# Brummi/MonoRec

Hardware: AMD Instinct MI355X
Metric: frames/sec (keyframes/s), KITTI 256x512 2-src/32-bin cost-volume inference (higher is better)
Workload: dtype f32

## Files before the change

### include/monorec_hip.h

```cpp
#ifndef MONOREC_HIP_H
#define MONOREC_HIP_H

#include <stddef.h>
#include <stdint.h>

#ifdef __cplusplus
extern "C" {
#endif

#define MR_ABI_VERSION 21

#define MR_COMPUTE_F32  0
#define MR_COMPUTE_BF16 1
#define MR_COMPUTE_BF16X3 2

#define MR_ERR_BAD_ARGUMENT (-1)
#define MR_ERR_UNSUPPORTED  (-2)
#define MR_ERR_LDS_BUDGET   (-3)

#define MR_MAX_SOURCES 3
#define MR_MAX_FRAMES  8
#define MR_MAX_HEADS   4
#define MR_MAX_VOTE_MASKS 8

enum {
    MR_ACT_NONE = 0,
    MR_ACT_RELU = 1,
    MR_ACT_LEAKY_RELU = 2,
    MR_ACT_SIGMOID = 3,
    MR_ACT_ABS_TANH_AFFINE = 4
};

enum {
    MR_IN_DIRECT = 0,
    MR_IN_UPSAMPLE2 = 1,
    MR_IN_MAXPOOL2 = 2
};

enum {
    MR_TF_NONE = 0,
    MR_TF_RESNET_NORM = 1
};

// ... 127 lines not shown
int mr_conv2d_b8(const mr_b8_conv_desc* desc, void* stream);
int mr_pool2x2_framemax_b8(const void* src, void* pooled, void* fmax, int32_t frames, int64_t planes, int32_t h, int32_t w, void* stream);
int mr_max_over_frames_b8(const void* src, void* dst, int32_t frames, int64_t groups16, void* stream);
int mr_cost_volume_b8_f32(const float* keyframe, const float* const* frames, int32_t num_frames, const float* kinv, const float* proj,
                          const float* depths, int32_t batch, int32_t num_depths, int32_t height, int32_t width, float alpha,
                          const float* channel_weights, int32_t use_ssim, const float* pixel_depths, float* cost_volume,
                          float* const* sfcv, void* const* sfcv_b8, void* stream);
int mr_cost_volume_b8_lean_f32(const float* keyframe, const float* const* frames, int32_t num_frames, const float* kinv, const float* proj,
                               const float* depths, int32_t batch, int32_t num_depths, int32_t height, int32_t width, float alpha,
                               const float* channel_weights, int32_t use_ssim, const float* pixel_depths, float* cost_volume,
                               float* const* sfcv_scratch, void* const* sfcv_b8, void* stream);
int mr_mask_classifier_b8_f32(const float* features, const float* weight, const float* bias, int32_t batch, int32_t channels, int64_t plane,
                              float* cv_mask, float* cost_volume, int32_t num_depths, void* cost_volume_b8, void* stream);
int mr_f32_nchw_to_b8(const float* src, void* dst, int32_t n, int32_t c, int64_t hw, void* stream);
int mr_b8_to_f32_nchw(const void* src, float* dst, int32_t n, int32_t c, int64_t hw, void* stream);

size_t mr_wino1d_packed_weight_floats(int32_t out_channels, const int32_t* src_channels, int32_t num_src, int32_t cout_blocks_per_wave);
int mr_wino1d_pack_weights_f32(const float* weight, int32_t out_channels, const int32_t* src_channels, int32_t num_src,
                               int32_t cout_blocks_per_wave, float* dst);
int64_t mr_conv1d3_winograd_lds_bytes(const mr_wino_desc* desc);
int mr_conv1d3_winograd_f32(const mr_wino_desc* desc, int32_t axis, void* stream);

size_t mr_cooktoom1d_packed_weight_floats(int32_t out_channels, const int32_t* src_channels, int32_t num_src, int32_t cout_blocks_per_wave,
                                          int32_t m, int32_t r);
int mr_cooktoom1d_pack_weights_f32(const float* weight, int32_t out_channels, const int32_t* src_channels, int32_t num_src,
                                   int32_t cout_blocks_per_wave, int32_t m, int32_t r, float* dst);
int64_t mr_conv1d_cooktoom_lds_bytes(const mr_wino_desc* desc, int32_t axis, int32_t m, int32_t r);
int mr_conv1d_cooktoom_f32(const mr_wino_desc* desc, int32_t axis, int32_t m, int32_t r, void* stream);

int mr_upconv_pack_weights_f32(const float* weight, int32_t out_channels, const int32_t* src_channels, int32_t num_src,
                               int32_t cout_blocks_per_wave, float* dst);
int mr_upconv2x2_winograd_f32(const mr_wino_desc* desc, void* stream);

size_t mr_wino_t_packed_weight_floats(int32_t out_channels, const int32_t* src_channels, int32_t num_src, int32_t cout_blocks_per_wave);
int mr_wino_t_pack_weights_f32(const float* weight, int32_t out_channels, const int32_t* src_channels, int32_t num_src,
                               int32_t cout_blocks_per_wave, float* dst);
size_t mr_wino_t_packed_weight_floats_tail(int32_t out_channels, const int32_t* src_channels, int32_t num_src);
int mr_wino_t_pack_weights_tail_f32(const float* weight, int32_t out_channels, const int32_t* src_channels, int32_t num_src, float* dst);
int64_t mr_convt4x4s2_winograd_lds_bytes(const mr_wino_desc* desc);
int mr_convt4x4s2_winograd_f32(const mr_wino_desc* desc, void* stream);

int mr_cost_volume_f32(const float* keyframe, const float* const* frames, int32_t num_frames,
                       const float* kinv, const float* proj, const float* depths,
                       int32_t batch, int32_t num_depths, int32_t height, int32_t width,
                       float alpha, const float* channel_weights ,
                       float* cost_volume, float* const* sfcv, void* stream);

int mr_cost_volume_mode_f32(const float* keyframe, const float* const* frames, int32_t num_frames,
                            const float* kinv, const float* proj, const float* depths,
                            int32_t batch, int32_t num_depths, int32_t height, int32_t width,
                            float alpha, const float* channel_weights, int32_t use_ssim,
                            const float* pixel_depths, int32_t sfcv_mult_mask,
                            float* cost_volume, float* const* sfcv, void* stream);

int mr_cost_volume_relaxed_f32(const float* keyframe, const float* const* frames, int32_t num_frames,
                               const float* kinv, const float* proj, const float* depths,
                               int32_t batch, int32_t num_depths, int32_t height, int32_t width,
                               float alpha, const float* channel_weights, int32_t use_ssim, const float* pixel_depths,
                               float* cost_volume, float* const* sfcv, void* stream);

int mr_cost_volume_tiled_f32(const float* keyframe, const float* const* frames, int32_t num_frames,
                             const float* kinv, const float* proj, const float* depths,
                             int32_t batch, int32_t num_depths, int32_t height, int32_t width,
                             float alpha, const float* channel_weights, int32_t use_ssim,
                             const float* pixel_depths, int32_t sfcv_mult_mask,
                             float* cost_volume, float* const* sfcv, void* stream);
// ... 132 lines not shown
```

### monorec_amd/_lib.py

```python
import ctypes
import os

MR_MAX_SOURCES = 3
MR_MAX_FRAMES = 8

ACT_NONE, ACT_RELU, ACT_LEAKY_RELU, ACT_SIGMOID, ACT_ABS_TANH_AFFINE = range(5)
IN_DIRECT, IN_UPSAMPLE2, IN_MAXPOOL2 = range(3)
TF_NONE, TF_RESNET_NORM = range(2)

_c_float_p = ctypes.POINTER(ctypes.c_float)


class ConvDesc(ctypes.Structure):
    _fields_ = [
        ("src", ctypes.c_void_p * MR_MAX_SOURCES),
        ("src_channels", ctypes.c_int32 * MR_MAX_SOURCES),
        ("num_src", ctypes.c_int32),
        ("batch", ctypes.c_int32),
        ("src_h", ctypes.c_int32), ("src_w", ctypes.c_int32),
        ("in_mode", ctypes.c_int32),
        ("in_transform", ctypes.c_int32),
        ("kh", ctypes.c_int32), ("kw", ctypes.c_int32),
        ("stride_h", ctypes.c_int32), ("stride_w", ctypes.c_int32),
        ("pad_top", ctypes.c_int32), ("pad_left", ctypes.c_int32),
# ... 24 lines not shown
        ("k_split_waves", ctypes.c_int32),
    ]


class WinoDesc(ctypes.Structure):
    _fields_ = [("src", ctypes.c_void_p * MR_MAX_SOURCES), ("src_channels", ctypes.c_int32 * MR_MAX_SOURCES), ("num_src", ctypes.c_int32),
                ("batch", ctypes.c_int32), ("height", ctypes.c_int32), ("width", ctypes.c_int32),
                ("dst", ctypes.c_void_p), ("out_channels", ctypes.c_int32),
                ("packed_weights", ctypes.c_void_p), ("bias", ctypes.c_void_p), ("residual", ctypes.c_void_p),
                ("activation", ctypes.c_int32), ("act_p0", ctypes.c_float), ("cout_blocks_per_wave", ctypes.c_int32),
                ("variant", ctypes.c_int32),
                ("src_row_pitch", ctypes.c_int32), ("src_plane_floats", ctypes.c_int32), ("dst_split_columns", ctypes.c_int32)]


LAYOUT_F32_NCHW, LAYOUT_BF16_B8 = 0, 1


class B8ConvDesc(ctypes.Structure):
    _fields_ = [("src", ctypes.c_void_p * MR_MAX_SOURCES), ("src_channels", ctypes.c_int32 * MR_MAX_SOURCES), ("src_layout", ctypes.c_int32 * MR_MAX_SOURCES),
                ("num_src", ctypes.c_int32), ("batch", ctypes.c_int32), ("src_h", ctypes.c_int32), ("src_w", ctypes.c_int32),
                ("kh", ctypes.c_int32), ("kw", ctypes.c_int32), ("stride_h", ctypes.c_int32), ("stride_w", ctypes.c_int32),
                ("out_h", ctypes.c_int32), ("out_w", ctypes.c_int32),
                ("dst", ctypes.c_void_p), ("dst_layout", ctypes.c_int32), ("out_channels", ctypes.c_int32),
                ("dst_plane_h", ctypes.c_int32), ("dst_plane_w", ctypes.c_int32), ("out_step_h", ctypes.c_int32), ("out_step_w", ctypes.c_int32),
                ("bias", ctypes.c_void_p), ("activation", ctypes.c_int32), ("act_p0", ctypes.c_float),
                ("cout_blocks_per_wg", ctypes.c_int32), ("pixel_blocks_per_wave", ctypes.c_int32), ("waves_per_wg", ctypes.c_int32),
                ("num_phases", ctypes.c_int32),
                ("phase_weights", ctypes.c_void_p * 4), ("phase_kh", ctypes.c_int32 * 4), ("phase_kw", ctypes.c_int32 * 4),
                ("phase_pad_top", ctypes.c_int32 * 4), ("phase_pad_left", ctypes.c_int32 * 4),
                ("phase_out_off_h", ctypes.c_int32 * 4), ("phase_out_off_w", ctypes.c_int32 * 4)]


MR_MAX_COPY_SEGMENTS = 24
MR_ABI_VERSION = 21


class CopySegment(ctypes.Structure):
    _fields_ = [("src", ctypes.c_void_p), ("dst", ctypes.c_void_p), ("bytes", ctypes.c_int64)]


class LaunchItem(ctypes.Structure):
    _fields_ = [("kind", ctypes.c_int32), ("arg", ctypes.c_int32), ("desc", ctypes.c_void_p)]


LAUNCH_CONV2D, LAUNCH_WINO3X3, LAUNCH_WINO_T, LAUNCH_WINO_1D, LAUNCH_UPCONV, LAUNCH_COOKTOOM_1D, LAUNCH_WINO44, LAUNCH_CONV_B8, LAUNCH_WINO44S, LAUNCH_WINO44W = 0, 1, 2, 3, 4, 5, 6, 7, 8, 9


class HeadDesc(ctypes.Structure):
    _fields_ = [("src", ctypes.c_void_p), ("weight", ctypes.c_void_p), ("bias", ctypes.c_void_p), ("dst", ctypes.c_void_p),
                ("batch", ctypes.c_int32), ("channels", ctypes.c_int32), ("height", ctypes.c_int32), ("width", ctypes.c_int32)]


MR_MAX_HEADS = 4

ABI = {
    "mr_conv_packed_weight_floats": (ctypes.c_size_t, [ctypes.c_int32, ctypes.POINTER(ctypes.c_int32), ctypes.c_int32,
                                                       ctypes.c_int32, ctypes.c_int32, ctypes.c_int32, ctypes.c_int32]),
    "mr_conv_pack_weights_f32": (ctypes.c_int, [ctypes.c_void_p, ctypes.c_int32, ctypes.POINTER(ctypes.c_int32),
                                                ctypes.c_int32, ctypes.c_int32, ctypes.c_int32, ctypes.c_int32,
                                                ctypes.c_int32, ctypes.c_void_p]),
    "mr_conv_packed_weight_floats_bf16": (ctypes.c_size_t, [ctypes.c_int32, ctypes.POINTER(ctypes.c_int32), ctypes.c_int32,
                                                            ctypes.c_int32, ctypes.c_int32, ctypes.c_int32, ctypes.c_int32]),
    "mr_conv_packed_weight_floats_bf16x3": (ctypes.c_size_t, [ctypes.c_int32, ctypes.POINTER(ctypes.c_int32), ctypes.c_int32,
                                                              ctypes.c_int32, ctypes.c_int32, ctypes.c_int32, ctypes.c_int32]),
    "mr_conv_pack_weights_bf16x3": (ctypes.c_int, [ctypes.c_void_p, ctypes.c_int32, ctypes.POINTER(ctypes.c_int32),
                                                    ctypes.c_int32, ctypes.c_int32, ctypes.c_int32, ctypes.c_int32, ctypes.c_int32,
                                                    ctypes.c_void_p]),
# ... 16 lines not shown
                                          ctypes.c_void_p, ctypes.c_void_p, ctypes.c_void_p,
                                          ctypes.c_int32, ctypes.c_int32, ctypes.c_int32, ctypes.c_int32,
                                          ctypes.c_float, _c_float_p,
                                          ctypes.c_void_p, ctypes.POINTER(ctypes.c_void_p), ctypes.c_void_p]),
    "mr_cost_volume_mode_f32": (ctypes.c_int, [ctypes.c_void_p, ctypes.POINTER(ctypes.c_void_p), ctypes.c_int32,
                                               ctypes.c_void_p, ctypes.c_void_p, ctypes.c_void_p,
                                               ctypes.c_int32, ctypes.c_int32, ctypes.c_int32, ctypes.c_int32,
                                               ctypes.c_float, _c_float_p, ctypes.c_int32, ctypes.c_void_p, ctypes.c_int32,
                                               ctypes.c_void_p, ctypes.POINTER(ctypes.c_void_p), ctypes.c_void_p]),
    "mr_cost_volume_relaxed_f32": (ctypes.c_int, [ctypes.c_void_p, ctypes.POINTER(ctypes.c_void_p), ctypes.c_int32,
                                                  ctypes.c_void_p, ctypes.c_void_p, ctypes.c_void_p,
                                                  ctypes.c_int32, ctypes.c_int32, ctypes.c_int32, ctypes.c_int32,
                                                  ctypes.c_float, _c_float_p, ctypes.c_int32, ctypes.c_void_p,
                                                  ctypes.c_void_p, ctypes.POINTER(ctypes.c_void_p), ctypes.c_void_p]),
    "mr_cost_volume_tiled_f32": (ctypes.c_int, [ctypes.c_void_p, ctypes.POINTER(ctypes.c_void_p), ctypes.c_int32,
                                                ctypes.c_void_p, ctypes.c_void_p, ctypes.c_void_p,
                                                ctypes.c_int32, ctypes.c_int32, ctypes.c_int32, ctypes.c_int32,
                                                ctypes.c_float, _c_float_p, ctypes.c_int32, ctypes.c_void_p, ctypes.c_int32,
                                                ctypes.c_void_p, ctypes.POINTER(ctypes.c_void_p), ctypes.c_void_p]),
    "mr_cost_volume_patch_f32": (ctypes.c_int, [ctypes.c_void_p, ctypes.POINTER(ctypes.c_void_p), ctypes.c_int32,
                                                ctypes.c_void_p, ctypes.c_void_p, ctypes.c_void_p,
                                                ctypes.c_int32, ctypes.c_int32, ctypes.c_int32, ctypes.c_int32,
                                                ctypes.c_float, _c_float_p, ctypes.c_int32, ctypes.c_void_p, ctypes.c_int32, ctypes.c_int32,
                                                ctypes.c_void_p, ctypes.POINTER(ctypes.c_void_p), ctypes.c_void_p]),
    "mr_maxpool3x3s2_f32": (ctypes.c_int, [ctypes.c_void_p, ctypes.c_void_p, ctypes.c_int32, ctypes.c_int32,
                                           ctypes.c_int32, ctypes.c_void_p]),
    "mr_maxpool2x2_f32": (ctypes.c_int, [ctypes.c_void_p, ctypes.c_void_p, ctypes.c_int64, ctypes.c_int32,
                                         ctypes.c_int32, ctypes.c_void_p]),
    "mr_resnet_normalize_f32": (ctypes.c_int, [ctypes.c_void_p, ctypes.c_void_p, ctypes.c_int64, ctypes.c_void_p]),
    "mr_exact_const_division": (ctypes.c_int, [ctypes.c_float]),
    "mr_run_launches": (ctypes.c_int, [ctypes.POINTER(LaunchItem), ctypes.c_int32, ctypes.c_void_p, ctypes.POINTER(ctypes.c_int32)]),
    "mr_upconv_pack_weights_f32": (ctypes.c_int, [ctypes.c_void_p, ctypes.c_int32, ctypes.POINTER(ctypes.c_int32), ctypes.c_int32, ctypes.c_int32, ctypes.c_void_p]),
    "mr_upconv2x2_winograd_f32": (ctypes.c_int, [ctypes.POINTER(WinoDesc), ctypes.c_void_p]),
    "mr_wino1d_packed_weight_floats": (ctypes.c_size_t, [ctypes.c_int32, ctypes.POINTER(ctypes.c_int32), ctypes.c_int32, ctypes.c_int32]),
    "mr_wino1d_pack_weights_f32": (ctypes.c_int, [ctypes.c_void_p, ctypes.c_int32, ctypes.POINTER(ctypes.c_int32), ctypes.c_int32, ctypes.c_int32, ctypes.c_void_p]),
    "mr_conv1d3_winograd_lds_bytes": (ctypes.c_int64, [ctypes.POINTER(WinoDesc)]),
    "mr_conv1d3_winograd_f32": (ctypes.c_int, [ctypes.POINTER(WinoDesc), ctypes.c_int32, ctypes.c_void_p]),
    "mr_cooktoom1d_packed_weight_floats": (ctypes.c_size_t, [ctypes.c_int32, ctypes.POINTER(ctypes.c_int32), ctypes.c_int32, ctypes.c_int32, ctypes.c_int32, ctypes.c_int32]),
    "mr_cooktoom1d_pack_weights_f32": (ctypes.c_int, [ctypes.c_void_p, ctypes.c_int32, ctypes.POINTER(ctypes.c_int32), ctypes.c_int32, ctypes.c_int32, ctypes.c_int32, ctypes.c_int32, ctypes.c_void_p]),
    "mr_conv1d_cooktoom_lds_bytes": (ctypes.c_int64, [ctypes.POINTER(WinoDesc), ctypes.c_int32, ctypes.c_int32, ctypes.c_int32]),
    "mr_conv1d_cooktoom_f32": (ctypes.c_int, [ctypes.POINTER(WinoDesc), ctypes.c_int32, ctypes.c_int32, ctypes.c_int32, ctypes.c_void_p]),
    "mr_wino_t_packed_weight_floats_tail": (ctypes.c_size_t, [ctypes.c_int32, ctypes.POINTER(ctypes.c_int32), ctypes.c_int32]),
    "mr_wino_t_pack_weights_tail_f32": (ctypes.c_int, [ctypes.c_void_p, ctypes.c_int32, ctypes.POINTER(ctypes.c_int32), ctypes.c_int32, ctypes.c_void_p]),
    "mr_wino_packed_weight_floats_tail": (ctypes.c_size_t, [ctypes.c_int32, ctypes.POINTER(ctypes.c_int32), ctypes.c_int32]),
    "mr_wino_pack_weights_tail_f32": (ctypes.c_int, [ctypes.c_void_p, ctypes.c_int32, ctypes.POINTER(ctypes.c_int32), ctypes.c_int32, ctypes.c_void_p]),
    "mr_b8_packed_weight_bytes": (ctypes.c_size_t, [ctypes.c_int32, ctypes.POINTER(ctypes.c_int32), ctypes.c_int32, ctypes.c_int32, ctypes.c_int32, ctypes.c_int32]),
    "mr_b8_pack_weights": (ctypes.c_int, [ctypes.c_void_p, ctypes.c_int32, ctypes.POINTER(ctypes.c_int32), ctypes.c_int32, ctypes.c_int32, ctypes.c_int32,
                                          ctypes.c_int32, ctypes.c_void_p]),
    "mr_conv2d_b8_lds_bytes": (ctypes.c_int64, [ctypes.POINTER(B8ConvDesc)]),
    "mr_conv2d_b8": (ctypes.c_int, [ctypes.POINTER(B8ConvDesc), ctypes.c_void_p]),
    "mr_pool2x2_framemax_b8": (ctypes.c_int, [ctypes.c_void_p, ctypes.c_void_p, ctypes.c_void_p, ctypes.c_int32, ctypes.c_int64, ctypes.c_int32,
                                              ctypes.c_int32, ctypes.c_void_p]),
    "mr_max_over_frames_b8": (ctypes.c_int, [ctypes.c_void_p, ctypes.c_void_p, ctypes.c_int32, ctypes.c_int64, ctypes.c_void_p]),
    "mr_f32_nchw_to_b8": (ctypes.c_int, [ctypes.c_void_p, ctypes.c_void_p, ctypes.c_int32, ctypes.c_int32, ctypes.c_int64, ctypes.c_void_p]),
    "mr_b8_to_f32_nchw": (ctypes.c_int, [ctypes.c_void_p, ctypes.c_void_p, ctypes.c_int32, ctypes.c_int32, ctypes.c_int64, ctypes.c_void_p]),
    "mr_cost_volume_b8_f32": (ctypes.c_int, [ctypes.c_void_p, ctypes.POINTER(ctypes.c_void_p), ctypes.c_int32, ctypes.c_void_p, ctypes.c_void_p,
                                             ctypes.c_void_p, ctypes.c_int32, ctypes.c_int32, ctypes.c_int32, ctypes.c_int32, ctypes.c_float, _c_float_p,
                                             ctypes.c_int32, ctypes.c_void_p, ctypes.c_void_p, ctypes.POINTER(ctypes.c_void_p),
                                             ctypes.POINTER(ctypes.c_void_p), ctypes.c_void_p]),
    "mr_cost_volume_b8_lean_f32": (ctypes.c_int, [ctypes.c_void_p, ctypes.POINTER(ctypes.c_void_p), ctypes.c_int32, ctypes.c_void_p, ctypes.c_void_p,
                                                  ctypes.c_void_p, ctypes.c_int32, ctypes.c_int32, ctypes.c_int32, ctypes.c_int32, ctypes.c_float, _c_float_p,
                                                  ctypes.c_int32, ctypes.c_void_p, ctypes.c_void_p, ctypes.POINTER(ctypes.c_void_p),
                                                  ctypes.POINTER(ctypes.c_void_p), ctypes.c_void_p]),
    "mr_mask_classifier_b8_f32": (ctypes.c_int, [ctypes.c_void_p, ctypes.c_void_p, ctypes.c_void_p, ctypes.c_int32, ctypes.c_int32, ctypes.c_int64,
                                                 ctypes.c_void_p, ctypes.c_void_p, ctypes.c_int32, ctypes.c_void_p, ctypes.c_void_p]),
    "mr_gather_small_f32": (ctypes.c_int, [ctypes.POINTER(ctypes.c_void_p), ctypes.c_int32, ctypes.c_int32, ctypes.c_void_p, ctypes.c_void_p]),
# ... 106 lines not shown
```

### monorec_amd/csrc/conv1d_wino.hip

```cpp
#include <hip/hip_runtime.h>
#include <math.h>
#include <string.h>

#include "../../include/monorec_hip.h"
#include "lds_dma.h"
#include "wino_host.h"

namespace {

constexpr int WCK = 8;
constexpr int RAW_PITCH = 40, RAW_ROWS = 10, RAW_PLANE = RAW_PITCH * RAW_ROWS;
constexpr int RAW_PLANE_X = 416;
static_assert(RAW_PLANE_X >= RAW_PLANE && RAW_PLANE_X % 64 == 32 && RAW_PLANE % 32 == 16, "plane pitches");
constexpr int NPOS = 4;

struct W1KArgs {
    const float* src[MR_MAX_SOURCES];
    int src_bytes[MR_MAX_SOURCES];
    int src_c[MR_MAX_SOURCES];
    int src_cpad[MR_MAX_SOURCES];
    int nsrc;
    int H, W;
    float* dst;
    const float* bias;
    int act;
    float p0;
    int Cout, tiles_x, nchunks;
    const float* w;
    long long wgroup_stride;
    int pitch, cplane;
    int dst_split;
    long long dst_half;
};

template <int AXIS, int MBW>
__global__ __launch_bounds__(512) void conv1d3_wino_kernel(const W1KArgs a) {
    extern __shared__ __attribute__((aligned(16))) float lds[];
    constexpr int U_FLOATS = NPOS * 2 * MBW * 64;
    constexpr int PLANE = AXIS == 0 ? RAW_PLANE_X : RAW_PLANE;
    constexpr int BUF = WCK * PLANE + U_FLOATS;
    const int tid = threadIdx.x;
    const int lane = tid & 63;
    const int wave = __builtin_amdgcn_readfirstlane(tid >> 6);
    const int ty_wg = (int)blockIdx.x / a.tiles_x, tx_wg = (int)blockIdx.x - ty_wg * a.tiles_x;
    const int grp = blockIdx.y, b = blockIdx.z;
    const int oy0 = ty_wg * 8, ox0 = tx_wg * 32;
    const int H = a.H, W = a.W, HW = H * W;

    int voff4[2];
#pragma unroll
    for (int i = 0; i < 2; ++i) {
        const int r = lane + 64 * i;
        const int row = r / 10, g4 = r - row * 10;
        const int gy = oy0 - 1 + row, gx = ox0 - 4 + 4 * g4;
        const bool inb = gy >= 0 && gy < H && gx >= 0 && gx < W;
        voff4[i] = r < RAW_ROWS * 10 ? (inb ? (gy * W + gx) * 4 : -1) : -2;
    }
    const unsigned lds_base = (unsigned)(unsigned long long)(__attribute__((address_space(3))) float*)lds;
    const float* wgrp = a.w + (long long)grp * a.wgroup_stride;

    f32x4 acc[NPOS][MBW];
#pragma unroll
    for (int p = 0; p < NPOS; ++p)
#pragma unroll
        for (int m = 0; m < MBW; ++m) acc[p][m] = (f32x4){0.f, 0.f, 0.f, 0.f};

    int cs = 0, cc0 = 0;
    auto issue = [&](int q, int pb) {
        const unsigned buf_addr = lds_base + pb * BUF * 4;
        const unsigned u_addr = buf_addr + WCK * PLANE * 4;
        const float* wsrc = wgrp + (long long)q * U_FLOATS;
        if (wave < U_FLOATS / 256) dma_global_x4(u_addr + wave * 1024, wsrc + wave * 256 + lane * 4);
        const i32x4 srd = make_srd(a.src[cs], a.src_bytes[cs]);
        const bool cok = cc0 + wave < a.src_c[cs];
        const int so = ((b * a.src_c[cs] + cc0 + (cok ? wave : 0)) * HW) * 4;
#pragma unroll
        for (int i = 0; i < 2; ++i)
            if (voff4[i] != -2) dma_buffer_x4(buf_addr + wave * (PLANE * 4) + i * 1024, cok ? voff4[i] : -1, srd, so);
        cc0 += WCK;
        if (cc0 >= a.src_cpad[cs]) { cc0 = 0; ++cs; }
    };

    issue(0, 0);
    const int t = lane & 15;
    const int patch0 = (lane >> 4) * PLANE + (AXIS == 0 ? (wave + 1) * RAW_PITCH + 2 * t + 2
                                                        : (2 * (wave >> 1)) * RAW_PITCH + 4 + (wave & 1) * 16 + t);
    for (int q = 0; q < a.nchunks; ++q) {
        const int pb = q & 1;
        const float* raw = lds + pb * BUF;
        const float* ub = raw + WCK * PLANE + lane;
        dma_wait_all();
        __syncthreads();
        if (q + 1 < a.nchunks) issue(q + 1, pb ^ 1);
        float v[2][NPOS];
#pragma unroll
        for (int c4 = 0; c4 < 2; ++c4) {
            const float* rp = raw + patch0 + c4 * 4 * PLANE;
            float d0, d1, d2, d3;
            if constexpr (AXIS == 0) {
                const f32x2 g0 = lds_pair(rp), g1 = lds_pair(rp + 2), g2 = lds_pair(rp + 4);
                d0 = g0.y; d1 = g1.x; d2 = g1.y; d3 = g2.x;
            } else {
                d0 = rp[0]; d1 = rp[RAW_PITCH]; d2 = rp[2 * RAW_PITCH]; d3 = rp[3 * RAW_PITCH];
            }
            v[c4][0] = d0 - d2;
            v[c4][1] = d1 + d2;
            v[c4][2] = d2 - d1;
            v[c4][3] = d1 - d3;
        }
#pragma unroll
        for (int p = 0; p < NPOS; ++p)
#pragma unroll
            for (int c4 = 0; c4 < 2; ++c4)
#pragma unroll
                for (int m = 0; m < MBW; ++m) {
                    const float av = ub[((p * 2 + c4) * MBW + m) * 64];
                    acc[p][m] = __builtin_amdgcn_mfma_f32_16x16x4f32(av, v[c4][p], acc[p][m], 0, 0, 0);
                }
    }
    const int ox = ox0 + (AXIS == 0 ? 2 * t : (wave & 1) * 16 + t);
    const int oy = oy0 + (AXIS == 0 ? wave : 2 * (wave >> 1));
    if (ox >= W || oy >= H) return;
#pragma unroll
    for (int m = 0; m < MBW; ++m)
#pragma unroll
        for (int r = 0; r < 4; ++r) {
// ... 77 lines not shown
        const int r = lane + 64 * i;
        const int row = r / Gm::G4, g4 = r - row * Gm::G4;
        const int gy = oy0 - (AXIS == 1 ? PL : 0) + row, gx = ox0 - 4 + 4 * g4;
        const bool inb = gy >= 0 && gy < H && gx >= 0 && gx < W;
        voff4[i] = r < Gm::NG ? (inb ? (gy * a.pitch + gx) * 4 : -1) : -2;
    }
    const unsigned lds_base = (unsigned)(unsigned long long)(__attribute__((address_space(3))) float*)lds;
    const float* wgrp = a.w + (long long)grp * a.wgroup_stride;

    f32x4 acc[N][MBW];
#pragma unroll
    for (int p = 0; p < N; ++p)
#pragma unroll
        for (int m = 0; m < MBW; ++m) acc[p][m] = (f32x4){0.f, 0.f, 0.f, 0.f};

    int cs = 0, cc0 = 0;
    auto issue = [&](int q, int pb) {
        const unsigned buf_addr = lds_base + pb * BUF * 4;
        const unsigned u_addr = buf_addr + WCK * PLANE * 4;
        const float* wsrc = wgrp + (long long)q * U_FLOATS;
#pragma unroll
        for (int pc = 0; pc < (U_PIECES + 7) / 8; ++pc)
            if (wave + 8 * pc < U_PIECES) dma_global_x4(u_addr + (wave + 8 * pc) * 1024, wsrc + (wave + 8 * pc) * 256 + lane * 4);
        const i32x4 srd = make_srd(a.src[cs], a.src_bytes[cs]);
        const bool cok = cc0 + wave < a.src_c[cs];
        const int so = ((b * a.src_c[cs] + cc0 + (cok ? wave : 0)) * HW) * 4;
#pragma unroll
        for (int i = 0; i < Gm::NI; ++i)
            if (voff4[i] != -2) dma_buffer_x4(buf_addr + wave * (PLANE * 4) + i * 1024, cok ? voff4[i] : -1, srd, so);
        cc0 += WCK;
        if (cc0 >= a.src_cpad[cs]) { cc0 = 0; ++cs; }
    };

    issue(0, 0);
    const int t = lane & 15;
    const int patch0 = (lane >> 4) * PLANE + (AXIS == 0 ? wave * PITCH + M * t : (M * (wave >> 1)) * PITCH + 4 + (wave & 1) * 16 + t);
    for (int q = 0; q < a.nchunks; ++q) {
        const int pb = q & 1;
        const float* raw = lds + pb * BUF;
        const float* ub = raw + WCK * PLANE + lane;
        dma_wait_all();
        __syncthreads();
        if (q + 1 < a.nchunks) issue(q + 1, pb ^ 1);
        float v[2][N];
#pragma unroll
        for (int c4 = 0; c4 < 2; ++c4) {
            const float* rp = raw + patch0 + c4 * 4 * PLANE;
            float d[N];
            if constexpr (AXIS == 1) {
#pragma unroll
                for (int i = 0; i < N; ++i) d[i] = rp[i * PITCH];
            } else if constexpr (M == 4) {
                float x[12];
#pragma unroll
                for (int j = 0; j < 3; ++j) {
                    const f32x4 g = *(const f32x4*)(rp + 4 * j);
                    x[4 * j] = g.x; x[4 * j + 1] = g.y; x[4 * j + 2] = g.z; x[4 * j + 3] = g.w;
                }
                static_assert(4 - PL + N <= 12, "three groups cover the patch");
#pragma unroll
                for (int i = 0; i < N; ++i) d[i] = x[4 - PL + i];
            } else {
                constexpr int NV = (4 - PL + N + 1) / 2;
                float x[2 * NV];
#pragma unroll
                for (int j = 0; j < NV; ++j) {
                    const float2 g = *(const float2*)(rp + 2 * j);
                    x[2 * j] = g.x; x[2 * j + 1] = g.y;
                }
#pragma unroll
                for (int i = 0; i < N; ++i) d[i] = x[4 - PL + i];
            }
            CtForm<M, R>::in(d, v[c4]);
        }
#pragma unroll
        for (int p = 0; p < N; ++p)
// ... 54 lines not shown
        const int r = lane + 64 * i;
        const int row = r / 10, g4 = r - row * 10;
        const int gy = iy0 - 1 + row, gx = ix0 - 4 + 4 * g4;
        const bool inb = gy >= 0 && gy < H && gx >= 0 && gx < W;
        voff4[i] = r < RAW_ROWS * 10 ? (inb ? (gy * W + gx) * 4 : -1) : -2;
    }
    const unsigned lds_base = (unsigned)(unsigned long long)(__attribute__((address_space(3))) float*)lds;
    const float* wgrp = a.w + (long long)grp * a.wgroup_stride;

    f32x4 acc[2][NPOS][MBW];
#pragma unroll
    for (int nb = 0; nb < 2; ++nb)
#pragma unroll
        for (int p = 0; p < NPOS; ++p)
#pragma unroll
            for (int m = 0; m < MBW; ++m) acc[nb][p][m] = (f32x4){0.f, 0.f, 0.f, 0.f};

    int cs = 0, cc0 = 0;
    auto issue = [&](int q, int pb) {
        const unsigned buf_addr = lds_base + pb * BUF * 4;
        const unsigned u_addr = buf_addr + WCK * RAW_PLANE * 4;
        const float* wsrc = wgrp + (long long)q * U_FLOATS;
        if (wave < U_FLOATS / 256) dma_global_x4(u_addr + wave * 1024, wsrc + wave * 256 + lane * 4);
        const i32x4 srd = make_srd(a.src[cs], a.src_bytes[cs]);
        const bool cok = cc0 + wave < a.src_c[cs];
        const int so = ((b * a.src_c[cs] + cc0 + (cok ? wave : 0)) * HW) * 4;
#pragma unroll
        for (int i = 0; i < 2; ++i)
            if (voff4[i] != -2) dma_buffer_x4(buf_addr + wave * (RAW_PLANE * 4) + i * 1024, cok ? voff4[i] : -1, srd, so);
        cc0 += WCK;
        if (cc0 >= a.src_cpad[cs]) { cc0 = 0; ++cs; }
    };

    issue(0, 0);
    const int t = lane & 15;
    const int patch0 = (lane >> 4) * RAW_PLANE + (wave + 1) * RAW_PITCH + 4 + t;
    for (int q = 0; q < a.nchunks; ++q) {
        const int pb = q & 1;
        const float* raw = lds + pb * BUF;
        const float* ub = raw + WCK * RAW_PLANE + lane;
        dma_wait_all();
        __syncthreads();
        if (q + 1 < a.nchunks) issue(q + 1, pb ^ 1);
        float v[2][2][NPOS];
#pragma unroll
        for (int nb = 0; nb < 2; ++nb)
#pragma unroll
            for (int c4 = 0; c4 < 2; ++c4) {
                const float* rp = raw + patch0 + c4 * 4 * RAW_PLANE + nb * 16;
                const float pa = rp[0], pb_ = rp[1], pc = rp[RAW_PITCH], pd = rp[RAW_PITCH + 1];
                v[nb][c4][0] = pa;
                v[nb][c4][1] = pb_ - pa;
                v[nb][c4][2] = pc - pa;
                v[nb][c4][3] = (pd - pb_) - (pc - pa);
            }
#pragma unroll
        for (int p = 0; p < NPOS; ++p)
#pragma unroll
            for (int c4 = 0; c4 < 2; ++c4)
#pragma unroll
                for (int m = 0; m < MBW; ++m) {
                    const float av = ub[((p * 2 + c4) * MBW + m) * 64];
#pragma unroll
                    for (int nb = 0; nb < 2; ++nb) acc[nb][p][m] = __builtin_amdgcn_mfma_f32_16x16x4f32(av, v[nb][c4][p], acc[nb][p][m], 0, 0, 0);
                }
    }
    const int iy = iy0 + wave;
    if (iy >= H) return;
    const int OW = 2 * W;
#pragma unroll
    for (int nb = 0; nb < 2; ++nb) {
        const int ix = ix0 + nb * 16 + t;
        if (ix >= W) continue;
#pragma unroll
        for (int m = 0; m < MBW; ++m)
#pragma unroll
            for (int r = 0; r < 4; ++r) {
                const int cout = (grp * MBW + m) * 16 + (lane >> 4) * 4 + r;
                if (cout >= a.Cout) continue;
                const float bs = a.bias ? a.bias[cout] : 0.f;
                const float m00 = acc[nb][0][m][r], m01 = acc[nb][1][m][r], m10 = acc[nb][2][m][r], m11 = acc[nb][3][m][r];
                const float o01 = m00 + m01;
                float* o = a.dst + ((long long)(b * a.Cout + cout) * (2 * H) + 2 * iy) * OW + 2 * ix;
                *(float2*)o = make_float2(act_max(m00 + bs, a.act, a.p0), act_max(o01 + bs, a.act, a.p0));
                *(float2*)(o + OW) = make_float2(act_max((m00 + m10) + bs, a.act, a.p0), act_max((o01 + (m10 + m11)) + bs, a.act, a.p0));
            }
    }
}

bool valid_mbw1(int m) { return m >= 1 && m <= 4; }

struct W1Derived {
    W1KArgs k;
    dim3 grid;
    size_t lds_bytes;
    int mbw;
};

int derive1(const mr_wino_desc* d, W1Derived* out, bool views = false) {
    if (const int rc = wino_check_shape(d)) return rc;
    if (!views && wino_is_view(d)) return MR_ERR_UNSUPPORTED;
    if (d->src_row_pitch < 0 || d->src_plane_floats < 0) return MR_ERR_BAD_ARGUMENT;
    const int pitch = d->src_row_pitch ? d->src_row_pitch : d->width;
    const long long cplane = d->src_plane_floats ? d->src_plane_floats : (long long)d->height * d->width;
    if (pitch < d->width || (pitch & 3) || cplane < (long long)(d->height - 1) * pitch + d->width || cplane >= (1ll << 30)) return MR_ERR_BAD_ARGUMENT;
    if (d->dst_split_columns && (d->width & 7)) return MR_ERR_UNSUPPORTED;
    if (d->residual) return MR_ERR_UNSUPPORTED;
    if (!valid_mbw1(d->cout_blocks_per_wave)) return MR_ERR_BAD_ARGUMENT;
    if (const int rc = wino_check_activation(d)) return rc;
    W1KArgs& k = out->k;
    int nchunks;
    if (const int rc = wino_fill_args(d, WCK, cplane, pitch - d->width, k, nchunks)) return rc;
    if (wino_dst_bytes(d) >= (1ll << 33)) return MR_ERR_UNSUPPORTED;
    k.pitch = pitch; k.cplane = (int)cplane;
    k.dst_split = d->dst_split_columns ? 1 : 0;
    k.dst_half = (long long)d->batch * d->out_channels * d->height * (d->width / 2);
    k.tiles_x = (d->width + 31) / 32;
    k.nchunks = nchunks;
    const int mbw = d->cout_blocks_per_wave;
    const int ufl = NPOS * 2 * mbw * 64;
    k.wgroup_stride = (long long)nchunks * ufl;
    const int groups = (d->out_channels + 16 * mbw - 1) / (16 * mbw);
    if (d->batch >= 65536 || groups >= 65536) return MR_ERR_UNSUPPORTED;
    out->grid = dim3((unsigned)(k.tiles_x * ((d->height + 7) / 8)), (unsigned)groups, (unsigned)d->batch);
    out->lds_bytes = (size_t)(2 * (WCK * RAW_PLANE_X + ufl)) * 4;
    out->mbw = mbw;
    return 0;
}

template <int AXIS, int MBW>
int launch1(const W1Derived& dv, hipStream_t stream) {
    hipLaunchKernelGGL((conv1d3_wino_kernel<AXIS, MBW>), dv.grid, dim3(512), dv.lds_bytes, stream, dv.k);
    return (int)hipGetLastError();
}

template <int AXIS>
int launch1_mbw(const W1Derived& dv, hipStream_t stream) {
    switch (dv.mbw) {
        case 1: return launch1<AXIS, 1>(dv, stream);
        case 2: return launch1<AXIS, 2>(dv, stream);
        case 3: return launch1<AXIS, 3>(dv, stream);
        default: return launch1<AXIS, 4>(dv, stream);
    }
}


#ifdef MR_DIAGNOSTIC_FORMS
bool valid_form(int m, int r) { return (m == 4 && r == 3) || (m == 2 && r == 7) || (m == 4 && r == 7) || (m == 4 && r == 4); }
#else
bool valid_form(int m, int r) { return (m == 4 && r == 3) || (m == 4 && r == 7) || (m == 4 && r == 4); }
#endif
bool valid_ct_mbw(int m, int r, int mbw) { return mbw >= 1 && mbw <= (m + r - 1 >= 10 ? 3 : 4); }

template <int AXIS, int M, int R>
int derive_ct_form(const mr_wino_desc* d, W1Derived* out) {
    using Gm = CtGeom<AXIS, M, R>;
    const int rc = derive1(d, out, true);
    if (rc != 0) return rc;
    if (d->dst_split_columns && AXIS != 1) return MR_ERR_UNSUPPORTED;
    const int mbw = d->cout_blocks_per_wave;
    const int ufl = ct_u_stream(Gm::N, mbw);
    out->k.tiles_x = (d->width + Gm::RW - 1) / Gm::RW;
    out->k.wgroup_stride = (long long)out->k.nchunks * ufl;
    out->grid = dim3((unsigned)(out->k.tiles_x * ((d->height + Gm::RH - 1) / Gm::RH)), out->grid.y, out->grid.z);
    out->lds_bytes = (size_t)(2 * (WCK * Gm::PLANE + ufl)) * 4;
    if (out->lds_bytes > 160 * 1024) return MR_ERR_LDS_BUDGET;
    return 0;
}

template <int AXIS, int MBW, int M, int R>
int launch_ct(const W1Derived& dv, hipStream_t stream) {
    return launch_lds_ceiling<conv1d_ct_kernel<AXIS, MBW, M, R>>(160 * 1024, dv.grid, dim3(512), dv.lds_bytes, stream, dv.k);
}

template <int AXIS, int M, int R>
int run_ct_form(const mr_wino_desc* d, hipStream_t stream, bool launch, int64_t* lds) {
    if (!d || !valid_ct_mbw(M, R, d->cout_blocks_per_wave)) return MR_ERR_BAD_ARGUMENT;
    W1Derived dv;
    const int rc = derive_ct_form<AXIS, M, R>(d, &dv);
    if (rc != 0) return rc;
    if (lds) *lds = (int64_t)dv.lds_bytes;
    if (!launch) return 0;
    switch (dv.mbw) {
        case 1: return launch_ct<AXIS, 1, M, R>(dv, stream);
        case 2: return launch_ct<AXIS, 2, M, R>(dv, stream);
        case 3: return launch_ct<AXIS, 3, M, R>(dv, stream);
        default:
            if constexpr (M + R - 1 < 10) return launch_ct<AXIS, 4, M, R>(dv, stream);
            else return MR_ERR_BAD_ARGUMENT;
    }
}

int run_ct(const mr_wino_desc* d, int axis, int m, int r, hipStream_t stream, bool launch, int64_t* lds) {
    if (!valid_form(m, r) || (axis != 0 && axis != 1)) return MR_ERR_BAD_ARGUMENT;
    if (m == 4 && r == 3) return axis == 0 ? run_ct_form<0, 4, 3>(d, stream, launch, lds) : run_ct_form<1, 4, 3>(d, stream, launch, lds);
    if (m == 4 && r == 4) return axis == 0 ? run_ct_form<0, 4, 4>(d, stream, launch, lds) : run_ct_form<1, 4, 4>(d, stream, launch, lds);
#ifdef MR_DIAGNOSTIC_FORMS
    if (m == 2 && r == 7) return axis == 0 ? run_ct_form<0, 2, 7>(d, stream, launch, lds) : run_ct_form<1, 2, 7>(d, stream, launch, lds);
#endif
    return axis == 0 ? run_ct_form<0, 4, 7>(d, stream, launch, lds) : run_ct_form<1, 4, 7>(d, stream, launch, lds);
}

const double* form_g(int m, int r) { return m == 4 && r == 3 ? CtForm<4, 3>::g() : m == 4 && r == 4 ? CtForm<4, 4>::g() : m == 2 ? CtForm<2, 7>::g() : CtForm<4, 7>::g(); }

}

extern "C" size_t mr_wino1d_packed_weight_floats(int32_t out_channels, const int32_t* src_channels, int32_t num_src, int32_t mbw) {
    if (!src_channels || num_src < 1 || num_src > MR_MAX_SOURCES || !valid_mbw1(mbw) || out_channels < 1) return 0;
    const int groups = (out_channels + 16 * mbw - 1) / (16 * mbw);
    return (size_t)groups * wino_chunks(src_channels, num_src) * (NPOS * 2 * mbw * 64);
}

extern "C" int mr_wino1d_pack_weights_f32(const float* weight, int32_t out_channels, const int32_t* src_channels, int32_t num_src,
                                          int32_t mbw, float* dst) {
    if (!weight || !dst || !src_channels || num_src < 1 || num_src > MR_MAX_SOURCES || !valid_mbw1(mbw) || out_channels < 1)
        return MR_ERR_BAD_ARGUMENT;
    const int cin_total = wino_sum_channels(src_channels, num_src);
    wino_pack_stream(dst, 0, out_channels, mbw, NPOS, 0, src_channels, num_src, [=](int cout, int cin, int p) {
        const float* gw = weight + ((size_t)cout * cin_total + cin) * 3;
        double u = 0.0;
        for (int i = 0; i < 3; ++i) u += WINO_G_2_3[p][i] * (double)gw[i];
        return u;
    });
    return 0;
}

extern "C" int64_t mr_conv1d3_winograd_lds_bytes(const mr_wino_desc* desc) {
    W1Derived dv;
    const int rc = derive1(desc, &dv);
    return rc != 0 ? rc : (int64_t)dv.lds_bytes;
}

extern "C" int mr_conv1d3_winograd_f32(const mr_wino_desc* desc, int32_t axis, void* stream) {
    W1Derived dv;
    const int rc = derive1(desc, &dv);
    if (rc != 0) return rc;
    if (axis == 0) return launch1_mbw<0>(dv, (hipStream_t)stream);
    if (axis == 1) return launch1_mbw<1>(dv, (hipStream_t)stream);
    return MR_ERR_BAD_ARGUMENT;
}

extern "C" size_t mr_cooktoom1d_packed_weight_floats(int32_t out_channels, const int32_t* src_channels, int32_t num_src, int32_t mbw,
                                                     int32_t m, int32_t r) {
    if (!src_channels || num_src < 1 || num_src > MR_MAX_SOURCES || !valid_form(m, r) || !valid_ct_mbw(m, r, mbw) || out_channels < 1) return 0;
    const int groups = (out_channels + 16 * mbw - 1) / (16 * mbw);
    return (size_t)groups * wino_chunks(src_channels, num_src) * ct_u_stream(m + r - 1, mbw);
}

extern "C" int mr_cooktoom1d_pack_weights_f32(const float* weight, int32_t out_channels, const int32_t* src_channels, int32_t num_src,
                                              int32_t mbw, int32_t m, int32_t r, float* dst) {
    if (!weight || !dst || !src_channels || num_src < 1 || num_src > MR_MAX_SOURCES || !valid_form(m, r) || !valid_ct_mbw(m, r, mbw) ||
        out_channels < 1)
        return MR_ERR_BAD_ARGUMENT;
    const double* G = form_g(m, r);
    const int npos = m + r - 1;
    const int cin_total = wino_sum_channels(src_channels, num_src);
// ... 6 lines not shown
    });
    return 0;
}

extern "C" int64_t mr_conv1d_cooktoom_lds_bytes(const mr_wino_desc* desc, int32_t axis, int32_t m, int32_t r) {
    int64_t lds = 0;
    const int rc = run_ct(desc, axis, m, r, nullptr, false, &lds);
    return rc != 0 ? rc : lds;
}

extern "C" int mr_conv1d_cooktoom_f32(const mr_wino_desc* desc, int32_t axis, int32_t m, int32_t r, void* stream) {
    return run_ct(desc, axis, m, r, (hipStream_t)stream, true, nullptr);
}

extern "C" int mr_upconv_pack_weights_f32(const float* weight, int32_t out_channels, const int32_t* src_channels, int32_t num_src,
                                          int32_t mbw, float* dst) {
    if (!weight || !dst || !src_channels || num_src < 1 || num_src > MR_MAX_SOURCES || !valid_mbw1(mbw) || out_channels < 1)
        return MR_ERR_BAD_ARGUMENT;
    const int cin_total = wino_sum_channels(src_channels, num_src);
    wino_pack_stream(dst, 0, out_channels, mbw, NPOS, 0, src_channels, num_src, [=](int cout, int cin, int p) {
        const float* gw = weight + ((size_t)cout * cin_total + cin) * 4;
        const double w00 = gw[0], w01 = gw[1], w10 = gw[2], w11 = gw[3];
        return p == 0 ? ((w00 + w01) + (w10 + w11)) : p == 1 ? (w01 + w11) : p == 2 ? (w10 + w11) : w11;
    });
    return 0;
}

extern "C" int mr_upconv2x2_winograd_f32(const mr_wino_desc* desc, void* stream) {
    W1Derived dv;
    const int rc = derive1(desc, &dv);
    if (rc != 0) return rc;
    if ((long long)desc->batch * desc->out_channels * desc->height * desc->width * 16 >= (1ll << 33)) return MR_ERR_UNSUPPORTED;
    if (dv.mbw > 2) return MR_ERR_BAD_ARGUMENT;
    if (dv.mbw == 1) hipLaunchKernelGGL((upconv2x2_wino_kernel<1>), dv.grid, dim3(512), dv.lds_bytes, (hipStream_t)stream, dv.k);
    else hipLaunchKernelGGL((upconv2x2_wino_kernel<2>), dv.grid, dim3(512), dv.lds_bytes, (hipStream_t)stream, dv.k);
    return (int)hipGetLastError();
}
```

### monorec_amd/csrc/lds_dma.h

```cpp
#pragma once
#include <hip/hip_runtime.h>

#include "../../include/monorec_hip.h"

typedef float f32x2 __attribute__((ext_vector_type(2)));
typedef float f32x4 __attribute__((ext_vector_type(4)));
typedef int i32x4 __attribute__((ext_vector_type(4)));

__device__ __forceinline__ void dma_buffer_x4(unsigned lds_byte_addr, int voff, i32x4 srd, int soff) {
    unsigned keep;
    lds_byte_addr = __builtin_amdgcn_readfirstlane(lds_byte_addr);
    soff = __builtin_amdgcn_readfirstlane(soff);
    asm volatile("s_nop 4\n\ts_mov_b32 %0, m0\n\ts_mov_b32 m0, %1\n\ts_nop 0\n\t"
                 "buffer_load_dwordx4 %2, %3, %4 offen lds\n\ts_mov_b32 m0, %0"
                 : "=&s"(keep) : "s"(lds_byte_addr), "v"(voff), "s"(srd), "s"(soff) : "memory");
}
__device__ __forceinline__ void dma_global_x4(unsigned lds_byte_addr, const void* g) {
    unsigned keep;
    lds_byte_addr = __builtin_amdgcn_readfirstlane(lds_byte_addr);
    asm volatile("s_nop 4\n\ts_mov_b32 %0, m0\n\ts_mov_b32 m0, %1\n\ts_nop 0\n\t"
                 "global_load_lds_dwordx4 %2, off\n\ts_mov_b32 m0, %0"
                 : "=&s"(keep) : "s"(lds_byte_addr), "v"(g) : "memory");
}
__device__ __forceinline__ void dma_global_x1(unsigned lds_byte_addr, const void* g) {
    unsigned keep;
    lds_byte_addr = __builtin_amdgcn_readfirstlane(lds_byte_addr);
    asm volatile("s_nop 4\n\ts_mov_b32 %0, m0\n\ts_mov_b32 m0, %1\n\ts_nop 0\n\t"
                 "global_load_lds_dword %2, off\n\ts_mov_b32 m0, %0"
                 : "=&s"(keep) : "s"(lds_byte_addr), "v"(g) : "memory");
}
__device__ __forceinline__ void dma_wait_all() { asm volatile("s_waitcnt vmcnt(0)" ::: "memory"); }
#define MR_VMCNT_CASE(N) case N: asm volatile("s_waitcnt vmcnt(" #N ")" ::: "memory"); break;
__device__ __forceinline__ void dma_wait_upto(int n) {
    switch (n < 32 ? n : (n < 48 ? 32 : 48)) {
        MR_VMCNT_CASE(0) MR_VMCNT_CASE(1) MR_VMCNT_CASE(2) MR_VMCNT_CASE(3) MR_VMCNT_CASE(4) MR_VMCNT_CASE(5) MR_VMCNT_CASE(6) MR_VMCNT_CASE(7)
        MR_VMCNT_CASE(8) MR_VMCNT_CASE(9) MR_VMCNT_CASE(10) MR_VMCNT_CASE(11) MR_VMCNT_CASE(12) MR_VMCNT_CASE(13) MR_VMCNT_CASE(14) MR_VMCNT_CASE(15)
        MR_VMCNT_CASE(16) MR_VMCNT_CASE(17) MR_VMCNT_CASE(18) MR_VMCNT_CASE(19) MR_VMCNT_CASE(20) MR_VMCNT_CASE(21) MR_VMCNT_CASE(22) MR_VMCNT_CASE(23)
        MR_VMCNT_CASE(24) MR_VMCNT_CASE(25) MR_VMCNT_CASE(26) MR_VMCNT_CASE(27) MR_VMCNT_CASE(28) MR_VMCNT_CASE(29) MR_VMCNT_CASE(30) MR_VMCNT_CASE(31)
        MR_VMCNT_CASE(32) MR_VMCNT_CASE(48)
        default: asm volatile("s_waitcnt vmcnt(0)" ::: "memory"); break;
    }
}

__device__ __forceinline__ i32x4 make_srd(const void* base, int bytes) {
    const unsigned long long p = (unsigned long long)base;
    i32x4 r;
    r.x = __builtin_amdgcn_readfirstlane((int)(unsigned)p);
    r.y = __builtin_amdgcn_readfirstlane((int)((unsigned)(p >> 32) & 0xffffu));
    r.z = __builtin_amdgcn_readfirstlane(bytes);
    r.w = 0x00020000;
    return r;
}

__device__ __forceinline__ f32x2 lds_pair(const float* p) {
    return *(const volatile __attribute__((address_space(3))) f32x2*)(__attribute__((address_space(3))) const float*)p;
}

__device__ __forceinline__ float act_max(float v, int act, float p0) {
    const unsigned keep = act == MR_ACT_RELU ? 0u : ~0u;
    const float lo = __uint_as_float(__float_as_uint(v * (act == MR_ACT_LEAKY_RELU ? p0 : 1.f)) & keep);
    return fmaxf(v, lo);
}
```

Measured before the change: 761.9.

## Generalize Winograd conv1d/Cook-Toom LDS double buffer into configurable multi-stage ring

Replaces the fixed two-stage LDS double buffer in the 1D Winograd, Cook-Toom and upconv kernels with an N-stage ring whose depth is chosen per launch. The choice depends on chunk count, grid size relative to CU count and an LDS budget. Partial vmcnt waits let several DMA stages stay in flight. The auto depth constant is 2, so the default behaviour equals the old double buffer; deeper rings only apply when forced through the new API. The change adds runtime ring index arithmetic, a CU-count query and a launch path with an LDS ceiling.

```diff
diff --git a/include/monorec_hip.h b/include/monorec_hip.h
--- a/include/monorec_hip.h
+++ b/include/monorec_hip.h
@@ -8,7 +8,7 @@
 extern "C" {
 #endif
 
-#define MR_ABI_VERSION 21
+#define MR_ABI_VERSION 22
 
 #define MR_COMPUTE_F32  0
 #define MR_COMPUTE_BF16 1
@@ -202,6 +202,8 @@
                                int32_t cout_blocks_per_wave, float* dst);
 int mr_upconv2x2_winograd_f32(const mr_wino_desc* desc, void* stream);
 
+int mr_wino_set_pipeline_depth(int32_t depth);
+
 size_t mr_wino_t_packed_weight_floats(int32_t out_channels, const int32_t* src_channels, int32_t num_src, int32_t cout_blocks_per_wave);
 int mr_wino_t_pack_weights_f32(const float* weight, int32_t out_channels, const int32_t* src_channels, int32_t num_src,
                                int32_t cout_blocks_per_wave, float* dst);
diff --git a/monorec_amd/_lib.py b/monorec_amd/_lib.py
--- a/monorec_amd/_lib.py
+++ b/monorec_amd/_lib.py
@@ -80,7 +80,7 @@
 
 
 MR_MAX_COPY_SEGMENTS = 24
-MR_ABI_VERSION = 21
+MR_ABI_VERSION = 22
 
 
 class CopySegment(ctypes.Structure):
@@ -163,6 +163,7 @@
     "mr_run_launches": (ctypes.c_int, [ctypes.POINTER(LaunchItem), ctypes.c_int32, ctypes.c_void_p, ctypes.POINTER(ctypes.c_int32)]),
     "mr_upconv_pack_weights_f32": (ctypes.c_int, [ctypes.c_void_p, ctypes.c_int32, ctypes.POINTER(ctypes.c_int32), ctypes.c_int32, ctypes.c_int32, ctypes.c_void_p]),
     "mr_upconv2x2_winograd_f32": (ctypes.c_int, [ctypes.POINTER(WinoDesc), ctypes.c_void_p]),
+    "mr_wino_set_pipeline_depth": (ctypes.c_int, [ctypes.c_int32]),
     "mr_wino1d_packed_weight_floats": (ctypes.c_size_t, [ctypes.c_int32, ctypes.POINTER(ctypes.c_int32), ctypes.c_int32, ctypes.c_int32]),
     "mr_wino1d_pack_weights_f32": (ctypes.c_int, [ctypes.c_void_p, ctypes.c_int32, ctypes.POINTER(ctypes.c_int32), ctypes.c_int32, ctypes.c_int32, ctypes.c_void_p]),
     "mr_conv1d3_winograd_lds_bytes": (ctypes.c_int64, [ctypes.POINTER(WinoDesc)]),
diff --git a/monorec_amd/csrc/conv1d_wino.hip b/monorec_amd/csrc/conv1d_wino.hip
--- a/monorec_amd/csrc/conv1d_wino.hip
+++ b/monorec_amd/csrc/conv1d_wino.hip
@@ -31,6 +31,7 @@
     int pitch, cplane;
     int dst_split;
     long long dst_half;
+    int depth;
 };
 
 template <int AXIS, int MBW>
@@ -81,17 +82,17 @@
         if (cc0 >= a.src_cpad[cs]) { cc0 = 0; ++cs; }
     };
 
-    issue(0, 0);
+    constexpr int NDMA = 2 + U_FLOATS / 256 / 8;
+    for (int j = 0; j < ring_prologue(a.depth, a.nchunks); ++j) issue(j, j);
     const int t = lane & 15;
     const int patch0 = (lane >> 4) * PLANE + (AXIS == 0 ? (wave + 1) * RAW_PITCH + 2 * t + 2
                                                         : (2 * (wave >> 1)) * RAW_PITCH + 4 + (wave & 1) * 16 + t);
-    for (int q = 0; q < a.nchunks; ++q) {
-        const int pb = q & 1;
+    for (int q = 0, pb = 0; q < a.nchunks; ++q, pb = ring_next(pb, a.depth)) {
         const float* raw = lds + pb * BUF;
         const float* ub = raw + WCK * PLANE + lane;
-        dma_wait_all();
+        ring_wait<NDMA>(q, a.nchunks, a.depth);
         __syncthreads();
-        if (q + 1 < a.nchunks) issue(q + 1, pb ^ 1);
+        if (q + a.depth - 1 < a.nchunks) issue(q + a.depth - 1, ring_prev(pb, a.depth));
         float v[2][NPOS];
 #pragma unroll
         for (int c4 = 0; c4 < 2; ++c4) {
@@ -235,16 +236,16 @@
         if (cc0 >= a.src_cpad[cs]) { cc0 = 0; ++cs; }
     };
 
-    issue(0, 0);
+    constexpr int NDMA = Gm::NI + U_PIECES / 8;
+    for (int j = 0; j < ring_prologue(a.depth, a.nchunks); ++j) issue(j, j);
     const int t = lane & 15;
     const int patch0 = (lane >> 4) * PLANE + (AXIS == 0 ? wave * PITCH + M * t : (M * (wave >> 1)) * PITCH + 4 + (wave & 1) * 16 + t);
-    for (int q = 0; q < a.nchunks; ++q) {
-        const int pb = q & 1;
+    for (int q = 0, pb = 0; q < a.nchunks; ++q, pb = ring_next(pb, a.depth)) {
         const float* raw = lds + pb * BUF;
         const float* ub = raw + WCK * PLANE + lane;
-        dma_wait_all();
+        ring_wait<NDMA>(q, a.nchunks, a.depth);
         __syncthreads();
-        if (q + 1 < a.nchunks) issue(q + 1, pb ^ 1);
+        if (q + a.depth - 1 < a.nchunks) issue(q + a.depth - 1, ring_prev(pb, a.depth));
         float v[2][N];
 #pragma unroll
         for (int c4 = 0; c4 < 2; ++c4) {
@@ -365,16 +366,16 @@
         if (cc0 >= a.src_cpad[cs]) { cc0 = 0; ++cs; }
     };
 
-    issue(0, 0);
+    constexpr int NDMA = 2 + U_FLOATS / 256 / 8;
+    for (int j = 0; j < ring_prologue(a.depth, a.nchunks); ++j) issue(j, j);
     const int t = lane & 15;
     const int patch0 = (lane >> 4) * RAW_PLANE + (wave + 1) * RAW_PITCH + 4 + t;
-    for (int q = 0; q < a.nchunks; ++q) {
-        const int pb = q & 1;
+    for (int q = 0, pb = 0; q < a.nchunks; ++q, pb = ring_next(pb, a.depth)) {
         const float* raw = lds + pb * BUF;
         const float* ub = raw + WCK * RAW_PLANE + lane;
-        dma_wait_all();
+        ring_wait<NDMA>(q, a.nchunks, a.depth);
         __syncthreads();
-        if (q + 1 < a.nchunks) issue(q + 1, pb ^ 1);
+        if (q + a.depth - 1 < a.nchunks) issue(q + a.depth - 1, ring_prev(pb, a.depth));
         float v[2][2][NPOS];
 #pragma unroll
         for (int nb = 0; nb < 2; ++nb)
@@ -422,6 +423,35 @@
 }
 
 bool valid_mbw1(int m) { return m >= 1 && m <= 4; }
+
+constexpr int RING_MAX_DEPTH = 6;
+constexpr int RING_AUTO_DEPTH = 2;
+constexpr int RING_WGS_PER_CU = 2;
+constexpr size_t RING_LDS_MAX = 160 * 1024;
+constexpr size_t CT_RING_AUTO_LDS = 112 * 1024;
+std::atomic<int> g_ring_depth{0};
+
+int device_cu_count() {
+    static std::atomic<int> cus{0};
+    int n = cus.load(std::memory_order_relaxed);
+    if (n) return n;
+    int dev = 0;
+    if (hipGetDevice(&dev) != hipSuccess || hipDeviceGetAttribute(&n, hipDeviceAttributeMultiprocessorCount, dev) != hipSuccess || n < 1) {
+        (void)hipGetLastError();
+        n = 256;
+    }
+    cus.store(n, std::memory_order_relaxed);
+    return n;
+}
+
+int ring_depth(int nchunks, long long wgs, size_t stage_bytes, size_t auto_cap) {
+    const int forced = g_ring_depth.load(std::memory_order_relaxed);
+    int depth = forced ? forced : (nchunks < 3 || wgs >= (long long)RING_WGS_PER_CU * device_cu_count() ? 2 : RING_AUTO_DEPTH);
+    const size_t cap = forced ? RING_LDS_MAX : auto_cap;
+    if (depth > nchunks) depth = nchunks;
+    while (depth > 2 && depth * stage_bytes > cap) --depth;
+    return depth < 2 ? 2 : depth;
+}
 
 struct W1Derived {
     W1KArgs k;
@@ -456,15 +486,16 @@
     const int groups = (d->out_channels + 16 * mbw - 1) / (16 * mbw);
     if (d->batch >= 65536 || groups >= 65536) return MR_ERR_UNSUPPORTED;
     out->grid = dim3((unsigned)(k.tiles_x * ((d->height + 7) / 8)), (unsigned)groups, (unsigned)d->batch);
-    out->lds_bytes = (size_t)(2 * (WCK * RAW_PLANE_X + ufl)) * 4;
+    const size_t stage = (size_t)(WCK * RAW_PLANE_X + ufl) * 4;
+    k.depth = ring_depth(nchunks, (long long)out->grid.x * out->grid.y * out->grid.z, stage, 64 * 1024);
+    out->lds_bytes = k.depth * stage;
     out->mbw = mbw;
     return 0;
 }
 
 template <int AXIS, int MBW>
 int launch1(const W1Derived& dv, hipStream_t stream) {
-    hipLaunchKernelGGL((conv1d3_wino_kernel<AXIS, MBW>), dv.grid, dim3(512), dv.lds_bytes, stream, dv.k);
-    return (int)hipGetLastError();
+    return launch_lds_ceiling<conv1d3_wino_kernel<AXIS, MBW>>((int)RING_LDS_MAX, dv.grid, dim3(512), dv.lds_bytes, stream, dv.k);
 }
 
 template <int AXIS>
@@ -496,8 +527,10 @@
     out->k.tiles_x = (d->width + Gm::RW - 1) / Gm::RW;
     out->k.wgroup_stride = (long long)out->k.nchunks * ufl;
     out->grid = dim3((unsigned)(out->k.tiles_x * ((d->height + Gm::RH - 1) / Gm::RH)), out->grid.y, out->grid.z);
-    out->lds_bytes = (size_t)(2 * (WCK * Gm::PLANE + ufl)) * 4;
-    if (out->lds_bytes > 160 * 1024) return MR_ERR_LDS_BUDGET;
+    const size_t stage = (size_t)(WCK * Gm::PLANE + ufl) * 4;
+    if (2 * stage > RING_LDS_MAX) return MR_ERR_LDS_BUDGET;
+    out->k.depth = ring_depth(out->k.nchunks, (long long)out->grid.x * out->grid.y * out->grid.z, stage, CT_RING_AUTO_LDS);
+    out->lds_bytes = out->k.depth * stage;
     return 0;
 }
 
@@ -555,6 +588,12 @@
         for (int i = 0; i < 3; ++i) u += WINO_G_2_3[p][i] * (double)gw[i];
         return u;
     });
+    return 0;
+}
+
+extern "C" int mr_wino_set_pipeline_depth(int32_t depth) {
+    if (depth != 0 && (depth < 2 || depth > RING_MAX_DEPTH)) return MR_ERR_BAD_ARGUMENT;
+    g_ring_depth.store(depth, std::memory_order_relaxed);
     return 0;
 }
 
@@ -627,7 +666,6 @@
     if (rc != 0) return rc;
     if ((long long)desc->batch * desc->out_channels * desc->height * desc->width * 16 >= (1ll << 33)) return MR_ERR_UNSUPPORTED;
     if (dv.mbw > 2) return MR_ERR_BAD_ARGUMENT;
-    if (dv.mbw == 1) hipLaunchKernelGGL((upconv2x2_wino_kernel<1>), dv.grid, dim3(512), dv.lds_bytes, (hipStream_t)stream, dv.k);
-    else hipLaunchKernelGGL((upconv2x2_wino_kernel<2>), dv.grid, dim3(512), dv.lds_bytes, (hipStream_t)stream, dv.k);
-    return (int)hipGetLastError();
-}
+    if (dv.mbw == 1) return launch_lds_ceiling<upconv2x2_wino_kernel<1>>((int)RING_LDS_MAX, dv.grid, dim3(512), dv.lds_bytes, (hipStream_t)stream, dv.k);
+    return launch_lds_ceiling<upconv2x2_wino_kernel<2>>((int)RING_LDS_MAX, dv.grid, dim3(512), dv.lds_bytes, (hipStream_t)stream, dv.k);
+}
diff --git a/monorec_amd/csrc/lds_dma.h b/monorec_amd/csrc/lds_dma.h
--- a/monorec_amd/csrc/lds_dma.h
+++ b/monorec_amd/csrc/lds_dma.h
@@ -42,6 +42,22 @@
     }
 }
 
+__device__ __forceinline__ int ring_prologue(int depth, int nchunks) { return depth - 1 < nchunks ? depth - 1 : nchunks; }
+__device__ __forceinline__ int ring_next(int stage, int depth) { return stage + 1 == depth ? 0 : stage + 1; }
+__device__ __forceinline__ int ring_prev(int stage, int depth) { return stage == 0 ? depth - 1 : stage - 1; }
+template <int N>
+__device__ __forceinline__ void ring_wait(int q, int nchunks, int depth) {
+    static_assert(N >= 1 && 4 * N <= 63, "vmcnt immediates of a ring of at most 6 stages");
+    const int behind = depth - 2 < nchunks - 1 - q ? depth - 2 : nchunks - 1 - q;
+    switch (behind) {
+        case 1: asm volatile("s_waitcnt vmcnt(%0)" ::"n"(N) : "memory"); break;
+        case 2: asm volatile("s_waitcnt vmcnt(%0)" ::"n"(2 * N) : "memory"); break;
+        case 3: asm volatile("s_waitcnt vmcnt(%0)" ::"n"(3 * N) : "memory"); break;
+        case 4: asm volatile("s_waitcnt vmcnt(%0)" ::"n"(4 * N) : "memory"); break;
+        default: dma_wait_all(); break;
+    }
+}
+
 __device__ __forceinline__ i32x4 make_srd(const void* base, int bytes) {
     const unsigned long long p = (unsigned long long)base;
     i32x4 r;
```

New measurement: 763.7 (median of 2 runs). No clear change (+0.2%).
